# s-will/BiAlign

Measured on AMD Instinct MI355X. Metric: giga-DP-cells/sec, higher is better.
Workload: dtype int32

## Files before the change

### bialign_amd/csrc/bialign_affine_point.hpp

```cpp
#pragma once

namespace bialign {

__device__ __forceinline__ int imax(int a, int b) { return a > b ? a : b; }
__device__ __forceinline__ int imin(int a, int b) { return a < b ? a : b; }
__device__ __forceinline__ int fM(int y, int x, int m) { return imax(imax(y, x), m); }
__device__ __forceinline__ int fX(int y, int x, int m, int beta) { return imax(x, beta + imax(y, m)); }
__device__ __forceinline__ int fY(int y, int x, int m, int beta) { return imax(y, beta + imax(x, m)); }

template <int W>
__host__ __device__ constexpr bool can_be_empty(int hU, int hV, int bb) {
  const int u0 = hU >= 1, u1 = hU != 1, v0 = hV >= 1, v1 = hV != 1;
  for (int aa = 0; aa < W; ++aa) {
    const int a1 = aa + u0 - v0, b1 = bb + u1 - v1;
    const int a2 = aa - v0, b2 = bb - v1;
    const int a3 = aa + u0, b3 = bb + u1;
    const bool g1 = a1 >= 0 && a1 < W && b1 >= 0 && b1 < W;
    const bool g2 = a2 >= 0 && a2 < W && b2 >= 0 && b2 < W;
    const bool g3 = a3 >= 0 && a3 < W && b3 >= 0 && b3 < W;
    if (!g1 && !g2 && !g3) return true;
  }
  return false;
}

template <bool V>
struct BoolTag {
  static constexpr bool value = V;
};

template <int W>
struct AffineCases {
  const int (&dA2)[2][W];
  const int& bb;
  const int (&dB)[4][W];
  const int (&dAx)[2][W];
  const int (&inB)[W][8];
  const int (&dC)[2][W];
  const int (&selfv)[4][W];
  const int &c_MM, &c_Mg, &c_gM, &gg, &ggdd;
  const int (&inC)[W][8];
  const int (&h2y)[3];
  const int &c2M, &gD, &c3M;

  __device__ __forceinline__ void operator()(int (&Tv)[9]) const {
#pragma unroll
    for (int hU = 0; hU < 3; ++hU) {
#pragma unroll
      for (int hV = 0; hV < 3; ++hV) {
        int gin = SENT;
        bool ok1 = true;
        if (hU == 2 && hV == 2) gin = dA2[0][bb];
        if (hU == 2 && hV == 1) { ok1 = bb + 1 < W; if (ok1) gin = dA2[1][bb + 1 < W ? bb + 1 : 0]; }
        if (hU == 2 && hV == 0) gin = dB[0][bb];
        if (hU == 1 && hV == 2) { ok1 = bb >= 1; if (ok1) gin = dAx[0][bb >= 1 ? bb - 1 : 0]; }
        if (hU == 1 && hV == 1) gin = dAx[1][bb];
        if (hU == 1 && hV == 0) { ok1 = bb >= 1; if (ok1) gin = inB[bb >= 1 ? bb - 1 : 0][1]; }
        if (hU == 0 && hV == 2) gin = dC[0][bb];
        if (hU == 0 && hV == 1) { ok1 = bb + 1 < W; if (ok1) gin = dC[1][bb + 1 < W ? bb + 1 : 0]; }
        if (hU == 0 && hV == 0) gin = selfv[0][bb];
        const int c1 = (hU == 2 && hV == 2) ? c_MM
                       : (hU == 2)          ? c_Mg
                       : (hV == 2)          ? c_gM
                       : (hU == hV)         ? gg
                                            : ggdd;
        int h2in = SENT;
        bool ok2 = true;
        if (hV == 2) { ok2 = bb >= 1; if (ok2) h2in = inC[bb >= 1 ? bb - 1 : 0][2 + hU]; }
        if (hV == 1) h2in = inC[bb][5 + hU];
        if (hV == 0) { ok2 = bb >= 1; if (ok2) h2in = h2y[hU]; }
        const int c2 = (hV == 2) ? c2M : gD;
        int h3in = SENT;
        bool ok3 = true;
        if (hU == 2) { ok3 = bb + 1 < W; if (ok3) h3in = dB[1 + hV][bb + 1 < W ? bb + 1 : 0]; }
        if (hU == 1) h3in = inB[bb][5 + hV];
        if (hU == 0) { ok3 = bb + 1 < W; if (ok3) h3in = selfv[1 + hV][bb + 1 < W ? bb + 1 : 0]; }
        const int c3 = (hU == 2) ? c3M : gD;

        int t = SENT;
        bool any = false;
        if (hU < 2 && hV < 2 && ok2 && ok3) {
          const int inner = ok1 ? imax(imax(gin + (c1 - gD), h2in), h3in) : imax(h2in, h3in);
          t = gD + inner;
        } else {
          if (ok1) { t = c1 + gin; any = true; }
          if (ok2) { t = any ? imax(t, c2 + h2in) : c2 + h2in; any = true; }
          if (ok3) { t = any ? imax(t, c3 + h3in) : c3 + h3in; any = true; }
        }
        Tv[3 * hU + hV] = t;
      }
    }
  }
};

template <int W>
__device__ __forceinline__ void dpp_from_left(const int r, int (&inC)[W][8], const int (&pubC)[W][8], const int lane_cap) {
  if (r + 1 < W) {
    asm("s_nop 1\n\t"
        "v_min_i32_dpp %0, %8, %16 wave_shr:1 row_mask:0xf bank_mask:0xf bound_ctrl:1\n\t"
        "v_min_i32_dpp %1, %9, %16 wave_shr:1 row_mask:0xf bank_mask:0xf bound_ctrl:1\n\t"
        "v_min_i32_dpp %2, %10, %16 wave_shr:1 row_mask:0xf bank_mask:0xf bound_ctrl:1\n\t"
        "v_min_i32_dpp %3, %11, %16 wave_shr:1 row_mask:0xf bank_mask:0xf bound_ctrl:1\n\t"
        "v_min_i32_dpp %4, %12, %16 wave_shr:1 row_mask:0xf bank_mask:0xf bound_ctrl:1\n\t"
        "v_min_i32_dpp %5, %13, %16 wave_shr:1 row_mask:0xf bank_mask:0xf bound_ctrl:1\n\t"
        "v_min_i32_dpp %6, %14, %16 wave_shr:1 row_mask:0xf bank_mask:0xf bound_ctrl:1\n\t"
        "v_min_i32_dpp %7, %15, %16 wave_shr:1 row_mask:0xf bank_mask:0xf bound_ctrl:1"
        : "=&v"(inC[r][0]), "=&v"(inC[r][1]), "=&v"(inC[r][2]), "=&v"(inC[r][3]), "=&v"(inC[r][4]),
          "=&v"(inC[r][5]), "=&v"(inC[r][6]), "=&v"(inC[r][7])
        : "v"(pubC[r][0]), "v"(pubC[r][1]), "v"(pubC[r][2]), "v"(pubC[r][3]), "v"(pubC[r][4]),
          "v"(pubC[r][5]), "v"(pubC[r][6]), "v"(pubC[r][7]), "v"(lane_cap));
  } else {
    asm("s_nop 1\n\t"
        "v_min_i32_dpp %0, %5, %10 wave_shr:1 row_mask:0xf bank_mask:0xf bound_ctrl:1\n\t"
        "v_min_i32_dpp %1, %6, %10 wave_shr:1 row_mask:0xf bank_mask:0xf bound_ctrl:1\n\t"
        "v_min_i32_dpp %2, %7, %10 wave_shr:1 row_mask:0xf bank_mask:0xf bound_ctrl:1\n\t"
        "v_min_i32_dpp %3, %8, %10 wave_shr:1 row_mask:0xf bank_mask:0xf bound_ctrl:1\n\t"
        "v_min_i32_dpp %4, %9, %10 wave_shr:1 row_mask:0xf bank_mask:0xf bound_ctrl:1"
        : "=&v"(inC[r][0]), "=&v"(inC[r][1]), "=&v"(inC[r][5]), "=&v"(inC[r][6]), "=&v"(inC[r][7])
        : "v"(pubC[r][0]), "v"(pubC[r][1]), "v"(pubC[r][5]), "v"(pubC[r][6]), "v"(pubC[r][7]), "v"(lane_cap));
    inC[r][2] = inC[r][3] = inC[r][4] = SENT;
  }
}

}
```

### bialign_amd/csrc/bialign_fill_slim.hpp

```cpp
#pragma once

namespace bialign {

template <int S, int TW, int PPW, bool LEAN = false>
__global__ void __launch_bounds__(64 * TW * PPW, 3) fill_affine_slim_kernel(const DeviceBatch A) {
  static_assert(S >= 1, "packed records need a band");
  using PK_ = Pack<S>;
  using G_ = Geo<S>;
  using R_ = Rec<S, 9, LEAN>;
  constexpr int W = G_::W, R = G_::R, RR = G_::RR, PADB = G_::PADB;
  constexpr int ND = R_::ND, NCH4 = R_::NCH4, TAIL = R_::TAIL, RECDW = R_::RECDW;
  static_assert(R * W < 64, "lane 63 must be free: it is the sentinel source of the exchange");
  extern __shared__ __align__(16) int32_t smem[];

  constexpr int T = TW;
  constexpr int NW = TW * PPW;
  const int L = threadIdx.x & 63;
  const int wv = NW == 1 ? 0 : __builtin_amdgcn_readfirstlane(threadIdx.x >> 6);
  const int pw = wv / TW, w = wv - pw * TW;
  const int slot = blockIdx.x * PPW + pw;
  const bool have_pair = slot < A.launch_pairs;
  const int pid = A.order[have_pair ? slot : 0];
  const PairDesc pd = A.pairs[pid];
  const int n = pd.n, m = pd.m, P = pd.P;
  const int il = L / W, aa = L - il * W;
  const bool live = L < R * W;
  const bool ghost = (il == 0);
  int ringfed_v = (ghost || !live) ? 1 : 0;
  asm volatile("" : "+v"(ringfed_v));
  const bool ringfed = ringfed_v != 0;
  int storing_v;
  {
    const int pad_idx0 = L < W ? L : (L >= R * W ? W + (L - R * W) : 64);
    storing_v = ((live && (LEAN ? il == R - 1 : !ghost)) || (!LEAN && pad_idx0 < R_::SLP - R_::SL)) ? 1 : 0;
  }
  asm volatile("" : "+v"(storing_v));
  const bool storing = storing_v != 0;
  const int beta = A.beta, gamma = A.gamma, delta = A.delta;
  const int k1 = A.k1, k2 = A.k2;
  const int gD = gamma + delta, gg = 2 * gamma, ggdd = 2 * gamma + 2 * delta, dd = 2 * delta;

  using GF = GhostFeed<S, 9, LEAN, 0>;
  constexpr int PERW = GF::RING_DW;
  constexpr int SENTBLK = 4 * GF::NP;
  v4i* ring = reinterpret_cast<v4i*>(smem + wv * GF::RING_DW);
  int32_t* sentblk = smem + NW * PERW;
  volatile int32_t* prog_lds = smem + NW * PERW + SENTBLK + pw * TW;
  const volatile int32_t* const fit_floor = smem + NW * PERW + SENTBLK + FIT_FLOOR_WORD;
  const volatile int32_t* const col0_floor = smem + NW * PERW + SENTBLK + COL0_FLOOR_WORD;
  int32_t* offtab = smem + NW * PERW + SENTBLK + LDS_PROG_WORDS;
  int32_t* s1 = offtab + slim_offtab_dw<S>();
  int32_t* s2 = s1 + k1 * k1;
  uint8_t* codes = reinterpret_cast<uint8_t*>(s2 + k2 * k2);
  const int npad = code_pad(n), mpad = code_pad(m, PADB);
  uint8_t* sa = codes + (size_t)pw * A.slim_code_bytes;
  uint8_t* ca = sa + npad;
  uint8_t* sb = ca + npad;
  uint8_t* cb = sb + mpad;

  for (int t = threadIdx.x; t < NW * PERW + SENTBLK; t += 64 * NW) smem[t] = SENT;
  if (threadIdx.x < LDS_PROG_WORDS) smem[NW * PERW + SENTBLK + threadIdx.x] = prog_word_init(threadIdx.x, A.free_ends);
  if (!LEAN)
    for (int t = threadIdx.x; t < GF::OFFTAB_DW; t += 64 * NW) offtab[t] = (int32_t)GF::lane_offset(t >> 6, t & 63);
  for (int t = threadIdx.x; t < k1 * k1; t += 64 * NW) s1[t] = A.s1[t];
  for (int t = threadIdx.x; t < k2 * k2; t += 64 * NW) s2[t] = A.s2[t];
  if (have_pair) {
    const int tt = threadIdx.x - pw * (64 * TW);
    for (int t = tt; t < n; t += 64 * TW) {
      sa[t] = A.seq_a[pd.seq_a + t];
      ca[t] = A.cls_a[pd.seq_a + t];
    }
    for (int t = tt; t < m + 2 * PADB; t += 64 * TW) {
      const int src = t - PADB;
      const bool ok = src >= 0 && src < m;
      sb[t] = ok ? A.seq_b[pd.seq_b + src] : 0;
      cb[t] = ok ? A.cls_b[pd.seq_b + src] : 0;
    }
  }
  __syncthreads();
  if (!have_pair) return;

  const int addrA = ((L - W) & 63) * 4;
  const int addrB = (live && aa < W - 1 ? ((L - W + 1) & 63) : 63) * 4;
  const bool a_first = (aa == 0);
  const int lane_cap = a_first ? SENT : 0x7fffffff;
  int32_t* const lay = A.layers + pd.layer_off;
  const int64_t pk_bnd_off = (int64_t)pd.G * PK_::RECDW;
  const int rec_last = pd.G - 1;
  const int NSw = (pd.NS - w + T - 1) / T;
  const int H = NSw > 0 ? (NSw - 1) * P + m + G_::MAXOFF + 1 : 0;

  int jj = -(2 * il + aa);
  int strip = 0;
  int rec_base = w * P;
  int i = 0, s1row = 0, s2row = 0;
  bool act_row = false;
  auto set_row = [&](int q) {
    i = (q * T + w) * RR + il - 1;
    const int k = i + aa - S;
    act_row = live && i >= 0 && i <= n && k >= 0 && k <= n;
    s1row = (i >= 1 && i <= n) ? sa[i - 1] * k1 : 0;
    s2row = (k >= 1 && k <= n) ? ca[k - 1] * k2 : 0;
  };
  set_row(0);

  int dA1[2][W], dA2[2][W];
  int dAx[2][W];
  int dB[4][W];
  int dC[2][W];
  int selfv[4][W];
  int pubC[W][8];
  int inC[W][8];
  int inA[W][4], inB[W][8];
#pragma unroll
  for (int bb = 0; bb < W; ++bb) {
    dA1[0][bb] = dA1[1][bb] = dA2[0][bb] = dA2[1][bb] = SENT;
    dAx[0][bb] = dAx[1][bb] = dC[0][bb] = dC[1][bb] = SENT;
#pragma unroll
    for (int x = 0; x < 4; ++x) dB[x][bb] = selfv[x][bb] = inA[bb][x] = SENT;
#pragma unroll
    for (int x = 0; x < 8; ++x) pubC[bb][x] = inB[bb][x] = inC[bb][x] = SENT;
  }
  const uint32_t ring_lds = __builtin_amdgcn_readfirstlane(
      (uint32_t)(uintptr_t)(__attribute__((address_space(3))) int32_t*)smem) + wv * GF::RING_DW * 4;

  using SA = StepAddr<S, LEAN>;
  using GS = GhostSrc<S, LEAN>;
  typedef const __attribute__((address_space(3))) int32_t* lds_cptr;
  typedef __attribute__((address_space(1))) char* gbl_ptr;
  typedef __attribute__((address_space(1))) v4i* gbl_v4i;
  typedef __attribute__((address_space(1))) int32_t* gbl_i32;
  uint32_t st_off = SA::chunk_off(L), st_toff = SA::tail_off(L), gs_fac = GS::factor(L);
  uint32_t gs_lane = GS::lane_byte(L, ring_lds + (NW - wv) * GF::RING_DW * 4);
  asm volatile("" : "+v"(st_off), "+v"(st_toff), "+v"(gs_fac), "+v"(gs_lane));
  int s_ph = 0, s_q = 0;
  int s_adv = 0;
  uint32_t ring_u = 0;
  gbl_ptr sbase = nullptr;

  int blk_q = 0, blk_rem = 0;
  int seen_prog = -0x40000000;
  auto wait_partner = [&](int h_last) __attribute__((always_inline)) {
    if (T == 1) return;
    const int src = w == 0 ? T - 1 : w - 1;
    const int need = h_last + 2 * (R - 1) + 1 - (w == 0 ? P : 0);
    if (seen_prog >= need) return;
    for (int spin = 0; (seen_prog = prog_lds[src]) < need; ++spin) {
      if (spin > A.spin_limit) {
        if (L == 0) atomicOr(A.errflag, 1);
        seen_prog = 0x7fffffff;
        break;
      }
      __builtin_amdgcn_s_sleep(16);
    }
  };
  bool blk_steady = false;
  auto prefetch_block = [&](int h0, int half) __attribute__((always_inline)) {
    wait_partner(h0 + GF::BLK - 1);
    if (!LEAN) blk_steady = GF::steady(blk_q, blk_rem, P, T, w, m, rec_last);
    int Lv = L;
    asm volatile("" : "+v"(Lv));
    if (!LEAN && blk_steady)
      GF::issue_steady(lay, blk_q, blk_rem, P, T, w, offtab, Lv, ring_lds + half * GF::SLOTS * 16);
    else if (LEAN) GF::issue(lay, h0, blk_q, blk_rem, P, T, w, P - 2 * (R - 1), rec_last, Lv, ring_lds + half * GF::SLOTS * 16);
    else GF::issue_packed(lay, pk_bnd_off, m, h0, blk_q, blk_rem, P, T, w, rec_last, Lv, ring_lds + half * GF::SLOTS * 16);
    blk_rem += GF::BLK;
    if (blk_rem >= P) { blk_rem -= P; ++blk_q; }
  };
  prefetch_block(0, 0);
  asm volatile("s_waitcnt vmcnt(0)" ::: "memory");
  int vm_younger = 0;
  int pk_all = 0;
  static_assert(LEAN || PK_::check_in_every_gap(GF::BLK),
                "range check: a test must fall into every non-interior stretch between two strips (pk_all is cleared, not kept, once a row leaves the lattice)");

  auto dmov = [](int& dst, int src) __attribute__((always_inline)) { asm("v_mov_b32 %0, %1" : "=v"(dst) : "v"(src)); };
  auto bperm = [](int addr, int v) __attribute__((always_inline)) -> int { return __builtin_amdgcn_ds_bpermute(addr, v); };

  int mu1n = 0, mu2n[W], sbn = 0, cbn = 0;
  auto lookup_mu = [&]() __attribute__((always_inline)) {
    const int jc = min(max(jj, 0), m + 1);
    mu1n = s1[s1row + sb[jc - 1 + PADB]];
#pragma unroll
    for (int bb = 0; bb < W; ++bb) mu2n[bb] = s2[s2row + cb[jc + bb]];
  };
  auto fetch_codes = [&](auto clamp_tag) __attribute__((always_inline)) {
    const int jc1 = decltype(clamp_tag)::value ? min(max(jj + 1, 0), m + 1) : jj + s_adv + 1;
    sbn = sb[jc1 - 1 + PADB];
    cbn = cb[jc1 + W - 1];
  };
  lookup_mu();
  fetch_codes(BoolTag<true>{});
  int fit_best = SENT, fit_j = 0;

  auto step = [&](auto interior_tag, int g) __attribute__((always_inline)) {
    constexpr bool INTERIOR = decltype(interior_tag)::value;
    if (!INTERIOR) {
      jj += s_adv;
      s_adv = 0;
    }
    const int gt = g & (GF::BLK - 1), ghalf = (g / GF::BLK) & 1;
    if (gt == 0) {
      GF::wait_block(vm_younger);
      if (TW > 1 && L == 0) prog_lds[w] = g - GF::BLK;
      if (!LEAN && (g & (PK_::CHECK - 1)) == 0) {
        const bool bad = live && !ghost && (unsigned)pk_all > 0xffffu;
        if (__builtin_amdgcn_ballot_w64(bad) != 0 && L == 0) atomicOr(A.errflag, 2);
        pk_all = 0;
      }
      if (!LEAN) {
        if (L < GF::BLK * W) {
          bool packed = true;
          if (!blk_steady) {
            int ph = s_ph + L / W, qst = s_q * T + w;
            if (ph >= P) { ph -= P; qst += T; }
            const int ts = ph + 2 * (R - 1), over = ts >= P ? 1 : 0;
            packed = PK_::interior(qst - 1 + over, ts - over * P, m);
          }
          if (packed) {
            v4i* pc = ring + ghalf * GF::SLOTS + L * GF::NP;
            int raw[4 * PK_::NPC], dec[4 * GF::NP];
#pragma unroll
            for (int c = 0; c < PK_::NPC; ++c) {
              const v4i v = pc[c];
              raw[4 * c] = v.x; raw[4 * c + 1] = v.y; raw[4 * c + 2] = v.z; raw[4 * c + 3] = v.w;
            }
#pragma unroll
            for (int d = 0; d < 4 * GF::NP; ++d) {
              const int h = PK_::hw(d < ND ? d : 0);
              const unsigned word = (unsigned)raw[d < ND && d != PK_::ANCHOR ? h >> 1 : 0];
              const unsigned e = d == PK_::ANCHOR ? 0x8000u : PK_::offset_of((h & 1) ? word >> 16 : word & 0xffffu, raw[0]);
              const int v = raw[0] + (int)e;
              dec[d] = d >= ND ? 0 : (pack_corner(W, d % 9, d / 9) ? (e == 0xffffu ? NEG : v) : v);
            }
#pragma unroll
            for (int c = 0; c < GF::NP; ++c) {
              v4i v;
              v.x = dec[4 * c]; v.y = dec[4 * c + 1]; v.z = dec[4 * c + 2]; v.w = dec[4 * c + 3];
              pc[c] = v;
            }
          }
        }
      }
      prefetch_block(g + GF::BLK, ghalf ^ 1);
      vm_younger = 0;
      ring_u = ring_lds + ghalf * GS::HALFB;
      if (A.prio_mode) {
        const int lvl = ((g >> 7) + (wv >> 2)) & 3;
        if (lvl == 0) __builtin_amdgcn_s_setprio(0);
        else if (lvl == 1) __builtin_amdgcn_s_setprio(1);
        else if (lvl == 2) __builtin_amdgcn_s_setprio(2);
        else __builtin_amdgcn_s_setprio(3);
      }
    }
    const int32_t* const gsrc = live ? reinterpret_cast<const int32_t*>(ring + ghalf * GF::SLOTS + (gt * W + aa) * GF::NP)
                                     : sentblk;
    uint32_t gaddr = 0;
    if (INTERIOR) asm("v_mad_u32_u24 %0, %1, %2, %3" : "=v"(gaddr) : "v"(gs_fac), "s"(ring_u), "v"(gs_lane));
    const lds_cptr gsrc_s = (lds_cptr)(uintptr_t)gaddr;
    auto at_store = [](uint32_t& off) __attribute__((always_inline)) -> uint32_t {
      asm volatile("" : "+v"(off));
      return off;
    };

    auto read_dpp = [&](int r) __attribute__((always_inline)) { dpp_from_left<W>(r, inC, pubC, lane_cap); };
    read_dpp(0);

    const int mu1 = mu1n;
    int mu2[W];
#pragma unroll
    for (int bb = 0; bb < W; ++bb) mu2[bb] = mu2n[bb];

    const bool tile_act = INTERIOR ? true : (act_row && jj >= 0 && jj <= m);
    const bool is_origin = INTERIOR ? false : (tile_act && i == 0 && jj == 0 && aa == S);
    const bool row0_diag = INTERIOR ? false : (tile_act && i == 0 && aa == S);
    const bool col0_diag = INTERIOR ? false : (tile_act && jj == 0 && aa == S);
    const int c3M = mu1 + dd, c_Mg = mu1 + gD;

    const int rec = g + rec_base;
    const int pad_idx = L < W ? L : (L >= R * W ? W + (L - R * W) : 64);
    const bool pad_lane = pad_idx < R_::SLP - R_::SL;
    constexpr bool PACKED = INTERIOR && !LEAN;
    const bool do_store = INTERIOR ? storing
                                   : (((live && (LEAN ? il == R - 1 : !ghost)) || (!LEAN && pad_lane)) &&
                                      __builtin_amdgcn_ballot_w64(tile_act && !ghost) != 0 && (TW == 1 || rec <= rec_last));
    const int slot_ = LEAN ? aa : (pad_lane ? R_::SL + pad_idx : L - W);
    if (INTERIOR) vm_younger += PACKED ? PK_::NPC : GF::STORES_PER_STEP;
    else if (__builtin_amdgcn_ballot_w64(do_store) != 0) vm_younger += GF::STORES_PER_STEP;
    int32_t* dst = lay + (int64_t)rec * RECDW;
    if (!INTERIOR && !LEAN) {
      const int tl = jj + 2 * il + aa;
      const int over = tl >= P ? 1 : 0;
      dst = lay + pk_bnd_off + PK_::bidx(strip * T + w + over, tl - over * P, P, m) * RECDW;
    }

    int outv[PACKED ? 1 : ND];
    int pk_base = 0, pk_min = 0, pk_max = 0, pk_e[PACKED ? ND : 1];
    int h2y[3] = {SENT, SENT, SENT};
    int defer[3] = {SENT, SENT, SENT};
#pragma unroll
    for (int bb = 0; bb < W; ++bb) {
      if (bb + 1 < W) read_dpp(bb + 1 < W ? bb + 1 : 0);
      const int l = jj + bb - S;
      const bool act = INTERIOR ? true : (tile_act && l >= 0 && l <= m);
      const int mu2v = mu2[bb];
      const int c_MM = mu1 + mu2v, c_gM = mu2v + gD, c2M = mu2v + dd;

      const AffineCases<W> cases{dA2, bb, dB, dAx, inB, dC, selfv, c_MM, c_Mg, c_gM, gg, ggdd, inC, h2y, c2M, gD, c3M};
      int M[9];
      bool isneg[9] = {};
      if (INTERIOR) {
        if (ringfed) {
#pragma unroll
          for (int q = 0; q < 9; ++q) M[q] = gsrc_s[bb * 9 + q];
        } else {
          int Tv[9];
          cases(Tv);
#pragma unroll
          for (int q = 0; q < 9; ++q) {
            int tv = Tv[q];
            if (can_be_empty<W>(q / 3, q % 3, bb)) {
              isneg[q] = tv < THRESH;
              tv = isneg[q] ? NEG : tv;
            }
            M[q] = tv;
          }
        }
      } else {
        int Gm[9];
#pragma unroll
        for (int q = 0; q < 9; ++q) Gm[q] = SENT;
        if (ghost) {
#pragma unroll
          for (int q = 0; q < 9; ++q) Gm[q] = gsrc[bb * 9 + q];
        }
        int Tv[9];
        cases(Tv);
        const int low = act ? NEG : SENT;
#pragma unroll
        for (int q = 0; q < 9; ++q) {
          const int tv = ghost ? Gm[q] : Tv[q];
          const bool bad = (tv < THRESH) | !act;
          M[q] = bad ? low : tv;
        }
        if (bb == S) M[8] = is_origin ? 0 : M[8];
        if (bb == S && row0_diag) M[8] = imax(M[8], fit_floor[0]);
        if (bb == S && col0_diag) M[8] = imax(M[8], col0_floor[0]);
      }
      if (!PACKED) {
#pragma unroll
        for (int q = 0; q < 9; ++q) outv[PACKED ? 0 : bb * 9 + q] = M[q];
      }
      if (LEAN && bb == S)
        lean_end_rule<INTERIOR>(A, pid, n, m, live && !ghost && aa == S, act_row, i, INTERIOR ? jj + s_adv : jj, fit_best,
                                fit_j, [&] {
          int best = M[0];
#pragma unroll
          for (int q = 1; q < 9; ++q) best = imax(best, M[q]);
          return best;
        });
      if (PACKED) {
        if (bb == 0) {
          pk_base = M[8] - 0x8000;
          pk_min = pk_max = M[8];
        }
        {
          int xs[9];
          int nx = 0;
#pragma unroll
          for (int q = 0; q < 9; ++q) {
            if (bb * 9 + q == PK_::ANCHOR) continue;
            int x = M[q];
            if (pack_corner(W, q, bb)) {
              const bool ng = isneg[q];
              x = ng ? pk_base + 0xffff : x;
            }
            pk_e[PACKED ? bb * 9 + q : 0] = x;
            xs[nx++] = x;
          }
#pragma unroll
          for (int t = 0; t + 1 < nx; t += 2) pk_min = imin(imin(pk_min, xs[t]), xs[t + 1]);
          if (nx & 1) pk_min = imin(pk_min, xs[nx - 1]);
        }
        if (do_store) {
#pragma unroll
          for (int c = 0; c < PK_::NPC; ++c) {
            constexpr int NDWc = PK_::NDW;
            const int dlast = 4 * c + 3 < NDWc - 1 ? 4 * c + 3 : NDWc - 1;
            const int last = PK_::val(2 * dlast + 1);
            if (last >= bb * 9 && last < (bb + 1) * 9) {
              int dw[4];
#pragma unroll
              for (int x = 0; x < 4; ++x) {
                const int d = 4 * c + x;
                const int lo = d < NDWc ? PK_::val(2 * d) : 0, hi = d < NDWc ? PK_::val(2 * d + 1) : 0;
                dw[x] = d == 0 ? pk_base
                               : (d < NDWc ? (int)__builtin_amdgcn_perm((unsigned)pk_e[PACKED ? hi : 0], (unsigned)pk_e[PACKED ? lo : 0], 0x05040100u) : 0);
              }
              if (c < PK_::NCH) {
                v4i v;
                v.x = dw[0]; v.y = dw[1]; v.z = dw[2]; v.w = dw[3];
                *reinterpret_cast<gbl_v4i>(sbase + SA::chunk_imm(c) + at_store(st_off)) = v;
              } else if (slot_ < PK_::TSLOTS) {
                const gbl_i32 tp = reinterpret_cast<gbl_i32>(sbase + SA::TAIL_IMM + at_store(st_toff));
#pragma unroll
                for (int x = 0; x < PK_::TAILDW; ++x) tp[x] = dw[x];
              }
            }
          }
        }
      } else {
        if (do_store) {
#pragma unroll
          for (int c = 0; c < NCH4; ++c) {
            if (4 * c + 3 >= bb * 9 && 4 * c + 3 < (bb + 1) * 9) {
              v4i v;
              v.x = outv[PACKED ? 0 : 4 * c]; v.y = outv[PACKED ? 0 : 4 * c + 1];
              v.z = outv[PACKED ? 0 : 4 * c + 2]; v.w = outv[PACKED ? 0 : 4 * c + 3];
              if (INTERIOR) *reinterpret_cast<gbl_v4i>(sbase + SA::chunk_imm(c) + at_store(st_off)) = v;
              else *reinterpret_cast<v4i*>(dst + c * R_::CH + slot_ * 4) = v;
            }
          }
          if (LEAN && bb == W - 1) {
            const gbl_i32 tp = INTERIOR ? reinterpret_cast<gbl_i32>(sbase + SA::TAIL_IMM + at_store(st_toff)) : nullptr;
#pragma unroll
            for (int t = 0; t < TAIL; ++t) {
              if (INTERIOR) tp[t] = outv[PACKED ? 0 : 4 * NCH4 + t];
              else dst[NCH4 * R_::CH + slot_ * TAIL + t] = outv[PACKED ? 0 : 4 * NCH4 + t];
            }
          }
        }
        if (!LEAN && bb == W - 1) {
          const bool wave_stores = __builtin_amdgcn_ballot_w64(tile_act && !ghost) != 0 && (TW == 1 || rec <= rec_last);
          if (wave_stores) {
            const int tslot = (live && !ghost) ? L - W : R_::SL + (L < W ? L : W + (L - R * W));
#pragma unroll
            for (int t = 0; t < TAIL; ++t) dst[NCH4 * R_::CH + tslot * TAIL + t] = outv[PACKED ? 0 : 4 * NCH4 + t];
          }
        }
      }

      int H2[3][3], H3[3][3], Gd[3][3];
#pragma unroll
      for (int u = 0; u < 3; ++u) {
        H2[u][2] = fM(M[3 * u], M[3 * u + 1], M[3 * u + 2]);
        const int bm = beta + H2[u][2];
        H2[u][0] = imax(M[3 * u], bm);
        H2[u][1] = imax(M[3 * u + 1], bm);
      }
#pragma unroll
      for (int v = 0; v < 3; ++v) {
        H3[2][v] = fM(M[v], M[3 + v], M[6 + v]);
        Gd[2][v] = fM(H2[0][v], H2[1][v], H2[2][v]);
        const int bm3 = beta + H3[2][v], bmg = beta + Gd[2][v];
        H3[0][v] = imax(M[v], bm3);
        H3[1][v] = imax(M[3 + v], bm3);
        Gd[0][v] = imax(H2[0][v], bmg);
        Gd[1][v] = imax(H2[1][v], bmg);
      }
      if (PACKED) {
        pk_max = imax(pk_max, Gd[2][2]);
        if (bb == W - 1) {
          const int acc = pk_all | (pk_max - pk_base + 1) | (pk_min - pk_base);
          pk_all = act_row ? acc : 0;
        }
      }
      pubC[bb][0] = Gd[0][2];
      pubC[bb][1] = Gd[0][1];
#pragma unroll
      for (int u = 0; u < 3; ++u) {
        pubC[bb][2 + u] = H2[u][2];
        pubC[bb][5 + u] = H2[u][1];
      }
      selfv[0][bb] = Gd[0][0];
#pragma unroll
      for (int v = 0; v < 3; ++v) selfv[1 + v][bb] = H3[0][v];
#pragma unroll
      for (int u = 0; u < 3; ++u) h2y[u] = H2[u][0];

      dmov(dA2[0][bb], dA1[0][bb]);
      dmov(dA2[1][bb], dA1[1][bb]);
      dmov(dA1[0][bb], inA[bb][0]);
      dmov(dA1[1][bb], inA[bb][1]);
      dmov(dB[0][bb], inB[bb][0]);
#pragma unroll
      for (int v = 0; v < 3; ++v) dmov(dB[1 + v][bb], inB[bb][2 + v]);
      dC[0][bb] = inC[bb][0];
      dC[1][bb] = inC[bb][1];
      inA[bb][0] = bperm(addrA, Gd[2][2]);
      inA[bb][1] = bperm(addrA, Gd[2][1]);
      inB[bb][0] = bperm(addrB, Gd[2][0]);
#pragma unroll
      for (int v = 0; v < 3; ++v) {
        inB[bb][2 + v] = bperm(addrB, H3[2][v]);
        inB[bb][5 + v] = bperm(addrB, H3[1][v]);
      }
      if (bb >= 1) {
        dmov(dAx[0][bb >= 1 ? bb - 1 : 0], inA[bb >= 1 ? bb - 1 : 0][2]);
        dmov(dAx[1][bb >= 1 ? bb - 1 : 0], inA[bb >= 1 ? bb - 1 : 0][3]);
        inA[bb >= 1 ? bb - 1 : 0][2] = bperm(addrA, defer[0]);
        inA[bb >= 1 ? bb - 1 : 0][3] = bperm(addrA, defer[1]);
        inB[bb >= 1 ? bb - 1 : 0][1] = bperm(addrB, defer[2]);
      }
      defer[0] = Gd[1][2];
      defer[1] = Gd[1][1];
      defer[2] = Gd[1][0];
    }
    dmov(dAx[0][W - 1], inA[W - 1][2]);
    dmov(dAx[1][W - 1], inA[W - 1][3]);
    inA[W - 1][2] = bperm(addrA, defer[0]);
    inA[W - 1][3] = bperm(addrA, defer[1]);
    inB[W - 1][1] = bperm(addrB, defer[2]);

    if (INTERIOR) ++s_adv;
    else ++jj;
    if (!INTERIOR && jj == P) {
      jj = 0;
      ++strip;
      rec_base += (T - 1) * P;
      set_row(strip);
    }
    ++s_ph;
    if (!INTERIOR && s_ph == P) {
      s_ph = 0;
      ++s_q;
    }
    ring_u += GS::STEPB;
    if (INTERIOR) {
      sbase += SA::RECB;
    } else {
      const uint64_t b = (uint64_t)(uintptr_t)(reinterpret_cast<char*>(lay) + SA::record_byte(g + 1, s_q, T, w, P));
      sbase = reinterpret_cast<gbl_ptr>((uintptr_t)((uint64_t)__builtin_amdgcn_readfirstlane((uint32_t)(b >> 32)) << 32 |
                                                    (uint32_t)__builtin_amdgcn_readfirstlane((uint32_t)b)));
    }
    if (INTERIOR) {
      mu1n = s1[s1row + sbn];
#pragma unroll
      for (int bb = 0; bb + 1 < W; ++bb) dmov(mu2n[bb], mu2[bb + 1]);
      mu2n[W - 1] = s2[s2row + cbn];
    } else {
      lookup_mu();
    }
    if (INTERIOR) fetch_codes(BoolTag<false>{});
    else fetch_codes(BoolTag<true>{});
  };

  auto all_interior = [&]() __attribute__((always_inline)) {
    (void)jj, (void)strip;
    return PK_::interior(s_q * T + w, s_ph, m);
  };
  int g = 0;
  while (g < H) {
    while (g < H && !all_interior()) {
      step(BoolTag<false>{}, g);
      ++g;
    }
    while (g < H && all_interior()) {
      step(BoolTag<true>{}, g);
      ++g;
    }
  }
  if (!LEAN && __builtin_amdgcn_ballot_w64(live && !ghost && (unsigned)pk_all > 0xffffu) != 0 && L == 0) atomicOr(A.errflag, 2);
  if (TW > 1) {
    asm volatile("s_waitcnt vmcnt(0)" ::: "memory");
    if (L == 0) prog_lds[w] = 0x7fffffff;
  }
}

}
```

Measured before the change: 213.6.

## Pre-add substitution costs into carried DP registers in interior steps

In interior steps, the substitution and gap cost addends are now folded into the carried registers (dA2, dB, dC, dAx) as they are moved, using v_add instead of v_mov. The inner max combinations in AffineCases can then skip those additions. Fold-in and fold-out passes adjust the registers when entering and leaving the interior phase. The change also replaces the tail store offset with a shift of the chunk offset to free a register, and moves code prefetching earlier. This trims per-cell ALU work, but the bookkeeping is intricate and the fold passes at phase transitions must invert each other exactly.

Result: no change. 214.9 (median of 6 runs) (+0.6%).

```diff
diff --git a/bialign_amd/csrc/bialign_affine_point.hpp b/bialign_amd/csrc/bialign_affine_point.hpp
--- a/bialign_amd/csrc/bialign_affine_point.hpp
+++ b/bialign_amd/csrc/bialign_affine_point.hpp
@@ -28,7 +28,7 @@
   static constexpr bool value = V;
 };
 
-template <int W>
+template <int W, bool FOLDED = false>
 struct AffineCases {
   const int (&dA2)[2][W];
   const int& bb;
@@ -78,13 +78,26 @@
 
         int t = SENT;
         bool any = false;
-        if (hU < 2 && hV < 2 && ok2 && ok3) {
-          const int inner = ok1 ? imax(imax(gin + (c1 - gD), h2in), h3in) : imax(h2in, h3in);
-          t = gD + inner;
+        if constexpr (!FOLDED) {
+          if (hU < 2 && hV < 2 && ok2 && ok3) {
+            const int inner = ok1 ? imax(imax(gin + (c1 - gD), h2in), h3in) : imax(h2in, h3in);
+            t = gD + inner;
+          } else {
+            if (ok1) { t = c1 + gin; any = true; }
+            if (ok2) { t = any ? imax(t, c2 + h2in) : c2 + h2in; any = true; }
+            if (ok3) { t = any ? imax(t, c3 + h3in) : c3 + h3in; any = true; }
+          }
         } else {
-          if (ok1) { t = c1 + gin; any = true; }
-          if (ok2) { t = any ? imax(t, c2 + h2in) : c2 + h2in; any = true; }
-          if (ok3) { t = any ? imax(t, c3 + h3in) : c3 + h3in; any = true; }
+          const bool pre1 = !(hU == 1 && hV == 0) && !(hU == 0 && hV == 0);
+          const bool pre3 = hU == 2;
+          if (hU < 2 && hV < 2 && ok2 && ok3) {
+            const int inner = ok1 ? imax(imax(pre1 ? gin : gin + (c1 - gD), h2in), h3in) : imax(h2in, h3in);
+            t = gD + inner;
+          } else {
+            if (ok1) { t = pre1 ? gin : c1 + gin; any = true; }
+            if (ok2) { t = any ? imax(t, c2 + h2in) : c2 + h2in; any = true; }
+            if (ok3) { const int g3 = pre3 ? h3in : c3 + h3in; t = any ? imax(t, g3) : g3; any = true; }
+          }
         }
         Tv[3 * hU + hV] = t;
       }
diff --git a/bialign_amd/csrc/bialign_fill_slim.hpp b/bialign_amd/csrc/bialign_fill_slim.hpp
--- a/bialign_amd/csrc/bialign_fill_slim.hpp
+++ b/bialign_amd/csrc/bialign_fill_slim.hpp
@@ -132,7 +132,9 @@
   typedef __attribute__((address_space(1))) int32_t* gbl_i32;
   uint32_t st_off = SA::chunk_off(L), st_toff = SA::tail_off(L), gs_fac = GS::factor(L);
   uint32_t gs_lane = GS::lane_byte(L, ring_lds + (NW - wv) * GF::RING_DW * 4);
-  asm volatile("" : "+v"(st_off), "+v"(st_toff), "+v"(gs_fac), "+v"(gs_lane));
+  asm volatile("" : "+v"(st_off), "+v"(gs_fac), "+v"(gs_lane));
+  static_assert(LEAN || SA::TAILB == 0 || SA::TAILB == 8 || SA::TAILB == 4, "tail_off = chunk_off * TAILB / 16 as a shift");
+  if (LEAN) asm volatile("" : "+v"(st_toff));
   int s_ph = 0, s_q = 0;
   int s_adv = 0;
   uint32_t ring_u = 0;
@@ -177,20 +179,22 @@
   auto dmov = [](int& dst, int src) __attribute__((always_inline)) { asm("v_mov_b32 %0, %1" : "=v"(dst) : "v"(src)); };
   auto bperm = [](int addr, int v) __attribute__((always_inline)) -> int { return __builtin_amdgcn_ds_bpermute(addr, v); };
 
-  int mu1n = 0, mu2n[W], sbn = 0, cbn = 0;
+  int mu1n = 0, mu2n[W], sbn = 0, cbn = 0, c2Mp = 0;
   auto lookup_mu = [&]() __attribute__((always_inline)) {
     const int jc = min(max(jj, 0), m + 1);
     mu1n = s1[s1row + sb[jc - 1 + PADB]];
 #pragma unroll
     for (int bb = 0; bb < W; ++bb) mu2n[bb] = s2[s2row + cb[jc + bb]];
   };
-  auto fetch_codes = [&](auto clamp_tag) __attribute__((always_inline)) {
-    const int jc1 = decltype(clamp_tag)::value ? min(max(jj + 1, 0), m + 1) : jj + s_adv + 1;
+  auto fetch_codes = [&]() __attribute__((always_inline)) {
+    const int jc1 = min(max(jj + 1, 0), m + 1);
     sbn = sb[jc1 - 1 + PADB];
     cbn = cb[jc1 + W - 1];
   };
+  auto wadd = [](int a, int b) __attribute__((always_inline)) -> int { return (int)((unsigned)a + (unsigned)b); };
+  auto wsub = [](int a, int b) __attribute__((always_inline)) -> int { return (int)((unsigned)a - (unsigned)b); };
   lookup_mu();
-  fetch_codes(BoolTag<true>{});
+  fetch_codes();
   int fit_best = SENT, fit_j = 0;
 
   auto step = [&](auto interior_tag, int g) __attribute__((always_inline)) {
@@ -261,6 +265,14 @@
     auto at_store = [](uint32_t& off) __attribute__((always_inline)) -> uint32_t {
       asm volatile("" : "+v"(off));
       return off;
+    };
+    auto last = [&](int& dst, int src, int addend) __attribute__((always_inline)) {
+      if (INTERIOR) asm("v_add_u32 %0, %1, %2" : "=v"(dst) : "v"(addend), "v"(src));
+      else dmov(dst, src);
+    };
+    auto lastk = [&](int& dst, int src, int addend) __attribute__((always_inline)) {
+      if (INTERIOR) asm("v_add_u32 %0, %1, %2" : "=v"(dst) : "s"(addend), "v"(src));
+      else dmov(dst, src);
     };
 
     auto read_dpp = [&](int r) __attribute__((always_inline)) { dpp_from_left<W>(r, inC, pubC, lane_cap); };
@@ -301,12 +313,14 @@
 #pragma unroll
     for (int bb = 0; bb < W; ++bb) {
       if (bb + 1 < W) read_dpp(bb + 1 < W ? bb + 1 : 0);
+      if (INTERIOR && bb == 0) cbn = cb[jj + s_adv + W + 1];
       const int l = jj + bb - S;
       const bool act = INTERIOR ? true : (tile_act && l >= 0 && l <= m);
-      const int mu2v = mu2[bb];
-      const int c_MM = mu1 + mu2v, c_gM = mu2v + gD, c2M = mu2v + dd;
-
-      const AffineCases<W> cases{dA2, bb, dB, dAx, inB, dC, selfv, c_MM, c_Mg, c_gM, gg, ggdd, inC, h2y, c2M, gD, c3M};
+      const int mu2a = mu2[bb];
+      const int mu2v = !INTERIOR ? mu2a : mu2[bb >= 1 ? bb - 1 : 0];
+      const int c_MM = mu1 + mu2a, c_gM0 = mu2a + gD, c2M = INTERIOR && bb == 0 ? c2Mp : mu2v + dd;
+
+      const AffineCases<W, INTERIOR> cases{dA2, bb, dB, dAx, inB, dC, selfv, c_MM, c_Mg, c_gM0, gg, ggdd, inC, h2y, c2M, gD, c3M};
       int M[9];
       bool isneg[9] = {};
       if (INTERIOR) {
@@ -402,7 +416,8 @@
                 v.x = dw[0]; v.y = dw[1]; v.z = dw[2]; v.w = dw[3];
                 *reinterpret_cast<gbl_v4i>(sbase + SA::chunk_imm(c) + at_store(st_off)) = v;
               } else if (slot_ < PK_::TSLOTS) {
-                const gbl_i32 tp = reinterpret_cast<gbl_i32>(sbase + SA::TAIL_IMM + at_store(st_toff));
+                uint32_t toff = st_off >> (SA::TAILB == 8 ? 1 : 2);
+                const gbl_i32 tp = reinterpret_cast<gbl_i32>(sbase + SA::TAIL_IMM + at_store(toff));
 #pragma unroll
                 for (int x = 0; x < PK_::TAILDW; ++x) tp[x] = dw[x];
               }
@@ -478,15 +493,22 @@
 #pragma unroll
       for (int u = 0; u < 3; ++u) h2y[u] = H2[u][0];
 
-      dmov(dA2[0][bb], dA1[0][bb]);
-      dmov(dA2[1][bb], dA1[1][bb]);
+      const int c_gM = INTERIOR ? wadd(mu2a, gD) : 0;
+      if (INTERIOR) asm("v_add3_u32 %0, %1, %2, %3" : "=v"(dA2[0][bb]) : "v"(dA1[0][bb]), "v"(mu1), "v"(mu2a));
+      else dmov(dA2[0][bb], dA1[0][bb]);
+      last(dA2[1][bb], dA1[1][bb], c_Mg);
       dmov(dA1[0][bb], inA[bb][0]);
       dmov(dA1[1][bb], inA[bb][1]);
-      dmov(dB[0][bb], inB[bb][0]);
-#pragma unroll
-      for (int v = 0; v < 3; ++v) dmov(dB[1 + v][bb], inB[bb][2 + v]);
-      dC[0][bb] = inC[bb][0];
-      dC[1][bb] = inC[bb][1];
+      last(dB[0][bb], inB[bb][0], c_Mg);
+#pragma unroll
+      for (int v = 0; v < 3; ++v) last(dB[1 + v][bb], inB[bb][2 + v], c3M);
+      if (INTERIOR) {
+        last(dC[0][bb], inC[bb][0], c_gM);
+        lastk(dC[1][bb], inC[bb][1], ggdd - gD);
+      } else {
+        dC[0][bb] = inC[bb][0];
+        dC[1][bb] = inC[bb][1];
+      }
       inA[bb][0] = bperm(addrA, Gd[2][2]);
       inA[bb][1] = bperm(addrA, Gd[2][1]);
       inB[bb][0] = bperm(addrB, Gd[2][0]);
@@ -496,8 +518,8 @@
         inB[bb][5 + v] = bperm(addrB, H3[1][v]);
       }
       if (bb >= 1) {
-        dmov(dAx[0][bb >= 1 ? bb - 1 : 0], inA[bb >= 1 ? bb - 1 : 0][2]);
-        dmov(dAx[1][bb >= 1 ? bb - 1 : 0], inA[bb >= 1 ? bb - 1 : 0][3]);
+        last(dAx[0][bb >= 1 ? bb - 1 : 0], inA[bb >= 1 ? bb - 1 : 0][2], c_gM);
+        lastk(dAx[1][bb >= 1 ? bb - 1 : 0], inA[bb >= 1 ? bb - 1 : 0][3], gg - gD);
         inA[bb >= 1 ? bb - 1 : 0][2] = bperm(addrA, defer[0]);
         inA[bb >= 1 ? bb - 1 : 0][3] = bperm(addrA, defer[1]);
         inB[bb >= 1 ? bb - 1 : 0][1] = bperm(addrB, defer[2]);
@@ -507,7 +529,7 @@
       defer[2] = Gd[1][0];
     }
     dmov(dAx[0][W - 1], inA[W - 1][2]);
-    dmov(dAx[1][W - 1], inA[W - 1][3]);
+    lastk(dAx[1][W - 1], inA[W - 1][3], gg - gD);
     inA[W - 1][2] = bperm(addrA, defer[0]);
     inA[W - 1][3] = bperm(addrA, defer[1]);
     inB[W - 1][1] = bperm(addrB, defer[2]);
@@ -535,19 +557,60 @@
     }
     if (INTERIOR) {
       mu1n = s1[s1row + sbn];
+      c2Mp = wadd(mu2[0], dd);
 #pragma unroll
       for (int bb = 0; bb + 1 < W; ++bb) dmov(mu2n[bb], mu2[bb + 1]);
       mu2n[W - 1] = s2[s2row + cbn];
+      sbn = sb[jj + s_adv + 1 + PADB];
     } else {
       lookup_mu();
     }
-    if (INTERIOR) fetch_codes(BoolTag<false>{});
-    else fetch_codes(BoolTag<true>{});
+    if (!INTERIOR) fetch_codes();
   };
 
   auto all_interior = [&]() __attribute__((always_inline)) {
     (void)jj, (void)strip;
     return PK_::interior(s_q * T + w, s_ph, m);
+  };
+  auto fold = [&](auto in_tag, const int mu1, const int (&mu2)[W]) __attribute__((always_inline)) {
+    constexpr bool IN = decltype(in_tag)::value;
+    auto app = [&](int& v, int addend) __attribute__((always_inline)) {
+      if (IN) asm("v_add_u32 %0, %0, %1" : "+v"(v) : "v"(addend));
+      else asm("v_sub_u32 %0, %0, %1" : "+v"(v) : "v"(addend));
+    };
+    const int c3M = wadd(mu1, dd), c_Mg = wadd(mu1, gD);
+#pragma unroll
+    for (int bb = 0; bb < W; ++bb) {
+      const int c_gM = wadd(mu2[bb], gD);
+      app(dA2[0][bb], wadd(mu1, mu2[bb]));
+      app(dB[0][bb], c_Mg);
+      app(dAx[1][bb], gg - gD);
+      app(dC[0][bb], c_gM);
+      if (bb >= 1) {
+        app(dA2[1][bb], c_Mg);
+#pragma unroll
+        for (int v = 0; v < 3; ++v) app(dB[1 + v][bb], c3M);
+        app(dAx[0][bb >= 1 ? bb - 1 : 0], c_gM);
+        app(dC[1][bb], ggdd - gD);
+      }
+    }
+  };
+  auto fold_in = [&]() __attribute__((always_inline)) {
+    fold(BoolTag<true>{}, mu1n, mu2n);
+    c2Mp = wadd(mu2n[0], dd);
+#pragma unroll
+    for (int bb = 0; bb + 1 < W; ++bb) mu2n[bb] = mu2n[bb + 1];
+    mu2n[W - 1] = s2[s2row + cbn];
+    mu1n = s1[s1row + sbn];
+    sbn = sb[jj + 1 + PADB];
+    asm volatile("" : "+v"(mu1n), "+v"(mu2n[W - 1]), "+v"(sbn));
+  };
+  auto fold_out = [&]() __attribute__((always_inline)) {
+#pragma unroll
+    for (int bb = W - 1; bb >= 1; --bb) mu2n[bb] = mu2n[bb - 1];
+    mu2n[0] = wsub(c2Mp, dd);
+    mu1n = s1[s1row + sb[jj + s_adv - 1 + PADB]];
+    fold(BoolTag<false>{}, mu1n, mu2n);
   };
   int g = 0;
   while (g < H) {
@@ -555,10 +618,13 @@
       step(BoolTag<false>{}, g);
       ++g;
     }
+    if (g >= H) break;
+    fold_in();
     while (g < H && all_interior()) {
       step(BoolTag<true>{}, g);
       ++g;
     }
+    fold_out();
   }
   if (!LEAN && __builtin_amdgcn_ballot_w64(live && !ghost && (unsigned)pk_all > 0xffffu) != 0 && L == 0) atomicOr(A.errflag, 2);
   if (TW > 1) {
```
